# Snoworday/instance-segmentation-attention

Measured on AMD Instinct MI355X. Metric: images/sec @256x256 bs=16 per GPU, higher is better.
Workload: dtype bf16; 1 GPU; train.py step fwd+bwd+update 256x256 bs=16/GPU (bf16); global_batch=16, parallelism=dp1, launch=hipGraph replay

## Files before the change

### instance-segmentation-attention_amd/csrc/conv_fused_bwd.hip

```cpp
#include "common.hpp"
#include "tr_lds.hpp"

int wgrad_slab_reduce_launch(float* ws, float* dw, float* dbias, int gx, int tn, int tk, int N, int cin, int taps,
                             isa_slab_arena* sa, hipStream_t s);

namespace {

struct PwParams {
    const bf16_t *g, *y, *x; bf16_t* dx; const float* w; float* dw;
    int N, K, ldg, ldy, ldx, lddx; long M;
    const float *ysc, *ysh, *ymu, *yis, *yred; float ycnt_inv; int yact; float *ydgamma, *ydbeta;
    const float *xsc, *xsh, *xmu, *xis; int xact; float* xred;
    int accumulate; float* ws;
    const bf16_t* addend; int lda;
    int G;
};

#ifdef ISA_PHASE_TRACE
__device__ unsigned long long phase_buf[10];
#endif

template <int TN, int TK, int YACT, int XMODE, bool EPI>
__global__ __launch_bounds__(256) __attribute__((amdgpu_waves_per_eu(2, 2))) void pw_bn_bwd_kernel(PwParams p) {
    extern __shared__ __attribute__((aligned(16))) char ldsb[];
    PHASE_DECL(); PHASE(0);
    constexpr int PMB = 32;
    constexpr int SN = TrStride<TN * 32>::bytes, SK = TrStride<TK * 32>::bytes;
    constexpr int SLAB = PMB * (SN + SK);
    constexpr int VN = TN * 4, VK = TK * 4;
    constexpr int LOADS_N = PMB * VN / 64, LOADS_K = PMB * VK / 64;
    constexpr int RPN = 64 / VN, RPK = 64 / VK;
    constexpr int XACT = XMODE == 1 ? ISA_ACT_RELU6 : (XMODE == 0 ? ISA_ACT_NONE : ACT_RT);
    constexpr int NS = TN * 2;
    const int tid = threadIdx.x, wave = tid >> 6, lane = tid & 63;
    const int r = lane & 31, hh = lane >> 5;
    char* sD = ldsb + wave * SLAB;
    char* sX = sD + PMB * SN;
    const GroupSel gs = group_sel(p.G);
    if (gs.g) {
        const long gm = (long)gs.g * p.M;
        p.g += gm * p.ldg; p.y += gm * p.ldy; p.x += gm * p.ldx; p.dx += gm * p.lddx;
        if (p.addend) p.addend += gm * p.lda;
        p.ysc += gs.g * p.N; p.ysh += gs.g * p.N; p.ymu += gs.g * p.N; p.yis += gs.g * p.N; p.yred += gs.g * ISA_STAT_R * 2 * p.N;
        p.xsc = goff(p.xsc, (long)gs.g * p.K); p.xsh = goff(p.xsh, (long)gs.g * p.K); p.xmu = goff(p.xmu, (long)gs.g * p.K);
        p.xis = goff(p.xis, (long)gs.g * p.K); p.xred = goff(p.xred, (long)gs.g * ISA_STAT_R * 2 * p.K);
    }
    const bool want_xred = XMODE == 1 || (XMODE == 2 && p.xred != nullptr);

    const int cgn = lane % VN, rown = lane / VN, cgk = lane % VK, rowk = lane / VK;
    const int cn0 = cgn * 8, ck0 = cgk * 8;
    const bool nok = cn0 < p.N, kok = ck0 < p.K;
    const int cnl = nok ? cn0 : 0, ckl = kok ? ck0 : 0;

    bf16x8 rg[LOADS_N], ry[LOADS_N], rx[LOADS_K], rxc[LOADS_K];
    const long nchunks = (p.M + PMB - 1) / PMB;
    auto fetch = [&](long chunk) {
        const long mbase = chunk * PMB;
#pragma unroll
        for (int v = 0; v < LOADS_N; ++v) {
            const long m = min(mbase + v * RPN + rown, p.M - 1);
            rg[v] = *reinterpret_cast<const bf16x8*>(p.g + m * p.ldg + cnl);
            ry[v] = *reinterpret_cast<const bf16x8*>(p.y + m * p.ldy + cnl);
        }
#pragma unroll
        for (int v = 0; v < LOADS_K; ++v) {
            const long m = min(mbase + v * RPK + rowk, p.M - 1);
            rx[v] = *reinterpret_cast<const bf16x8*>(p.x + m * p.ldx + ckl);
        }
    };
    const long stride = (long)gs.nbx * 4;
    long chunk = (long)gs.bx * 4 + wave;
    if (chunk < nchunks) fetch(chunk);

    float* cst = reinterpret_cast<float*>(ldsb + 4 * SLAB);
    constexpr int WP = TN * 32 + 8;
    bf16_t* wl = reinterpret_cast<bf16_t*>(ldsb);
    float wv[TN * TK * 4];
#pragma unroll
    for (int it = 0; it < TN * TK * 4; ++it) {
        const int i = it * 256 + tid, n = i / (TK * 32), k = i % (TK * 32);
        wv[it] = p.w[min(n, p.N - 1) * p.K + min(k, p.K - 1)];
    }
    if (tid < 64) {
        const int cn = min(tid, p.N - 1), ck = min(tid, p.K - 1);
        cst[0 * 64 + tid] = p.ysc[cn]; cst[1 * 64 + tid] = p.ysh[cn]; cst[2 * 64 + tid] = p.ymu[cn];
        float r0 = 0.f, r1 = 0.f;
#pragma unroll
        for (int r = 0; r < ISA_STAT_R; ++r) { r0 += p.yred[r * 2 * p.N + cn]; r1 += p.yred[r * 2 * p.N + p.N + cn]; }
        cst[3 * 64 + tid] = p.yis[cn] * (r1 * p.ycnt_inv);
        cst[4 * 64 + tid] = r0 * p.ycnt_inv;
        if (gs.bx == 0 && tid < p.N) {
            if (p.ydgamma) atomicAdd(p.ydgamma + tid, r1);
            if (p.ydbeta) atomicAdd(p.ydbeta + tid, r0);
        }
        cst[5 * 64 + tid] = (XMODE && p.xsc) ? p.xsc[ck] : 1.f; cst[6 * 64 + tid] = (XMODE && p.xsh) ? p.xsh[ck] : 0.f;
        cst[7 * 64 + tid] = (XMODE && p.xmu) ? p.xmu[ck] : 0.f; cst[8 * 64 + tid] = (XMODE && p.xis) ? p.xis[ck] : 1.f;
    }
#pragma unroll
    for (int it = 0; it < TN * TK * 4; ++it) {
        const int i = it * 256 + tid, n = i / (TK * 32), k = i % (TK * 32);
        wl[k * WP + n] = (bf16_t)((n < p.N && k < p.K) ? wv[it] : 0.f);
    }
    __syncthreads();
    PHASE(1);
    auto ldc = [&](int which, int c0, float (&v)[8]) {
        const f32x4 a = *reinterpret_cast<const f32x4*>(cst + which * 64 + c0), b = *reinterpret_cast<const f32x4*>(cst + which * 64 + c0 + 4);
#pragma unroll
        for (int j = 0; j < 4; ++j) { v[j] = a[j]; v[4 + j] = b[j]; }
    };
    bf16x8 wb[NS][TK];
#pragma unroll
    for (int s = 0; s < NS; ++s)
#pragma unroll
        for (int j = 0; j < TK; ++j)
            wb[s][j] = *reinterpret_cast<const bf16x8*>(wl + (32 * j + r) * WP + 16 * s + 8 * hh);
    __syncthreads();
    PHASE(2);

    f32x16 acc[TN][TK];
#pragma unroll
    for (int i = 0; i < TN; ++i)
#pragma unroll
        for (int j = 0; j < TK; ++j) acc[i][j] = f32x16{0};
    float s0[8], s1[8];
#pragma unroll
    for (int j = 0; j < 8; ++j) { s0[j] = 0.f; s1[j] = 0.f; }

    auto stash = [&](long chunk) {
        const long mbase = chunk * PMB;
        {
        float ysc[8], ysh[8], ymu[8], yq[8], yk0[8];
        ldc(0, cn0, ysc); ldc(1, cn0, ysh); ldc(2, cn0, ymu); ldc(3, cn0, yq); ldc(4, cn0, yk0);
#pragma unroll
        for (int v = 0; v < LOADS_N; ++v) {
            const bool ok = (mbase + v * RPN + rown) < p.M && nok;
            bf16x8 o;
#pragma unroll
            for (int j = 0; j < 8; ++j) {
                const float yy = (float)ry[v][j];
                const float dz = (float)rg[v][j] * act_grad_t<YACT>(fmaf(yy, ysc[j], ysh[j]), p.yact);
                const float val = ysc[j] * (dz - yk0[j] - (yy - ymu[j]) * yq[j]);
                o[j] = (bf16_t)((ok && cn0 + j < p.N) ? val : 0.f);
            }
            *reinterpret_cast<bf16x8*>(sD + (v * RPN + rown) * SN + cgn * 16) = o;
        }
        }
        float xsc[8], xsh[8];
        ldc(5, ck0, xsc); ldc(6, ck0, xsh);
#pragma unroll
        for (int v = 0; v < LOADS_K; ++v) {
            const bool ok = (mbase + v * RPK + rowk) < p.M && kok;
            bf16x8 o;
#pragma unroll
            for (int j = 0; j < 8; ++j) {
                const float xr = (float)rx[v][j];
                const float z = XMODE ? act_t<XACT>(fmaf(xr, xsc[j], xsh[j]), p.xact) : xr;
                o[j] = (bf16_t)((ok && ck0 + j < p.K) ? z : 0.f);
            }
            *reinterpret_cast<bf16x8*>(sX + (v * RPK + rowk) * SK + cgk * 16) = o;
            rxc[v] = rx[v];
        }
    };

    for (; chunk < nchunks; chunk += stride) {
        stash(chunk);
        __builtin_amdgcn_fence(__ATOMIC_RELEASE, "wavefront");
        __builtin_amdgcn_wave_barrier();
        PHASE_ONCE(3);
        constexpr bool EPI_PREFETCH = EPI && TK == 1;
        bf16x8 repi_old[EPI_PREFETCH ? LOADS_K : 1], repi_add[EPI_PREFETCH ? LOADS_K : 1];
        if constexpr (EPI_PREFETCH) {
            const long mb = chunk * PMB;
#pragma unroll
            for (int v = 0; v < LOADS_K; ++v) {
                const long m = min(mb + v * RPK + rowk, p.M - 1);
                repi_old[v] = bf16x8{0}; repi_add[v] = bf16x8{0};
                if (p.accumulate) repi_old[v] = *reinterpret_cast<const bf16x8*>(p.dx + m * p.lddx + ckl);
                if (p.addend) repi_add[v] = *reinterpret_cast<const bf16x8*>(p.addend + m * p.lda + ckl);
            }
        }
        if (chunk + stride < nchunks) fetch(chunk + stride);
#pragma unroll
        for (int s = 0; s < PMB / 16; ++s) {
            bf16x8 a[TN], b[TK];
#pragma unroll
            for (int i = 0; i < TN; ++i) a[i] = tr_frag(sD, SN, 16 * s, i * 32, lane);
#pragma unroll
            for (int j = 0; j < TK; ++j) b[j] = tr_frag(sX, SK, 16 * s, j * 32, lane);
#pragma unroll
            for (int i = 0; i < TN; ++i)
#pragma unroll
                for (int j = 0; j < TK; ++j)
                    acc[i][j] = __builtin_amdgcn_mfma_f32_32x32x16_bf16(a[i], b[j], acc[i][j], 0, 0, 0);
        }
        f32x16 dxa[TK];
#pragma unroll
        for (int j = 0; j < TK; ++j) dxa[j] = f32x16{0};
#pragma unroll
        for (int s = 0; s < NS; ++s) {
            const bf16x8 a = *reinterpret_cast<const bf16x8*>(sD + r * SN + (16 * s + 8 * hh) * 2);
#pragma unroll
            for (int j = 0; j < TK; ++j)
                dxa[j] = __builtin_amdgcn_mfma_f32_32x32x16_bf16(a, wb[s][j], dxa[j], 0, 0, 0);
        }
        __builtin_amdgcn_fence(__ATOMIC_RELEASE, "wavefront");
        __builtin_amdgcn_wave_barrier();
#pragma unroll
        for (int j = 0; j < TK; ++j)
#pragma unroll
            for (int e = 0; e < 16; ++e) {
                const int row = (e & 3) + 8 * (e >> 2) + 4 * hh;
                *reinterpret_cast<bf16_t*>(sX + row * SK + (32 * j + r) * 2) = (bf16_t)dxa[j][e];
            }
        __builtin_amdgcn_fence(__ATOMIC_RELEASE, "wavefront");
        __builtin_amdgcn_wave_barrier();
        const long mbase = chunk * PMB;
        float xsc[8], xsh[8], xmu[8], xis[8];
        if (want_xred) { ldc(5, ck0, xsc); ldc(6, ck0, xsh); ldc(7, ck0, xmu); ldc(8, ck0, xis); }
#pragma unroll
        for (int v = 0; v < LOADS_K; ++v) {
            const long m = mbase + v * RPK + rowk;
            if (m < p.M && kok) {
                bf16x8 o = *reinterpret_cast<const bf16x8*>(sX + (v * RPK + rowk) * SK + cgk * 16);
                bf16_t* dst = p.dx + m * p.lddx + ck0;
                if constexpr (EPI) {
                    if (p.accumulate) {
                        bf16x8 old;
                        if constexpr (EPI_PREFETCH) old = repi_old[v]; else old = *reinterpret_cast<const bf16x8*>(dst);
#pragma unroll
                        for (int j = 0; j < 8; ++j) o[j] = (bf16_t)((float)o[j] + (float)old[j]);
                    }
                    if (p.addend) {
                        bf16x8 ad;
                        if constexpr (EPI_PREFETCH) ad = repi_add[v]; else ad = *reinterpret_cast<const bf16x8*>(p.addend + m * p.lda + ck0);
#pragma unroll
                        for (int j = 0; j < 8; ++j) o[j] = (bf16_t)((float)o[j] + (float)ad[j]);
                    }
                }
                *reinterpret_cast<bf16x8*>(dst) = o;
                if (want_xred) {
#pragma unroll
                    for (int j = 0; j < 8; ++j) {
                        const float xr = (float)rxc[v][j];
                        const float dz = (float)o[j] * act_grad_t<XACT>(fmaf(xr, xsc[j], xsh[j]), p.xact);
                        s0[j] += dz; s1[j] += dz * ((xr - xmu[j]) * xis[j]);
                    }
                }
            }
        }
        __builtin_amdgcn_fence(__ATOMIC_RELEASE, "wavefront");
        __builtin_amdgcn_wave_barrier();
    }

    PHASE(4);
    __syncthreads();
    PHASE(5);
    float* part = reinterpret_cast<float*>(ldsb);
    float* xs = part + fold_part_floats<TN, TK>();
    fold_park<TN, TK>(part, acc, wave, lane);
    if (want_xred) {
        float* slot = xs + (wave * 4 + (lane >> 4)) * (2 * TK * 32);
#pragma unroll
        for (int j = 0; j < 8; ++j) {
            const float v0 = row_fold<VK>(s0[j]), v1 = row_fold<VK>(s1[j]);
            if ((lane & 15) < VK) { slot[ck0 + j] = v0; slot[TK * 32 + ck0 + j] = v1; }
        }
    }
    __syncthreads();
    PHASE(6);
    constexpr int SLABF = TN * TK * 1024 + TN * 32;
    float* slab = p.ws + (long)blockIdx.x * SLABF;
    fold_store<TN, TK>(part, slab, tid);
    PHASE(7);
    if (tid < TN * 32) slab[TN * TK * 1024 + tid] = 0.f;
    if (want_xred && tid < 2 * TK * 32) {
        float v = 0.f;
#pragma unroll
        for (int sl = 0; sl < 16; ++sl) v += xs[sl * (2 * TK * 32) + tid];
        const int which = tid / (TK * 32), c = tid - which * TK * 32;
        if (c < p.K && v != 0.f)
            atomicAdd(p.xred + (blockIdx.x & (ISA_STAT_R - 1)) * 2 * p.K + which * p.K + c, v);
    }
    PHASE(8);
    PHASE_FLUSH(phase_buf);
}

template <int TN, int TK, int YACT, int XMODE>
int launch_inst(PwParams& p, long ws_floats, isa_slab_arena* sa, const isa_pro* xfin, int xfin_groups, hipStream_t s) {
    constexpr int SN = TrStride<TN * 32>::bytes, SK = TrStride<TK * 32>::bytes;
    constexpr size_t slab = (size_t)32 * (SN + SK) * 4 + 9 * 64 * 4;
    constexpr size_t redb = ((size_t)fold_part_floats<TN, TK>() + 16 * 2 * TK * 32) * 4;
    constexpr size_t lds = slab > redb ? slab : redb;
    const long nchunks = (p.M + 31) / 32;
    const long slabf = (long)TN * TK * 1024 + TN * 32;
    long gx = (nchunks + 3) / 4 * p.G;
    if (gx > 256 * 2) gx = 256 * 2;
    if (int rc = defer_ws(sa, &p.ws, &ws_floats)) return rc;
    const long ws_cap = ws_floats / slabf;
    if (ws_cap < p.G) return sa ? ISA_ENOMEM : ISA_EINVAL;
    if (gx > ws_cap) gx = ws_cap;
    gx = group_grid(gx, p.G);
    if (int rc = fin_standalone(xfin, p.K, xfin_groups, s)) return rc;
    if (p.accumulate || p.addend) hipLaunchKernelGGL((pw_bn_bwd_kernel<TN, TK, YACT, XMODE, true>), dim3((unsigned)gx), dim3(256), lds, s, p);
    else hipLaunchKernelGGL((pw_bn_bwd_kernel<TN, TK, YACT, XMODE, false>), dim3((unsigned)gx), dim3(256), lds, s, p);
    if (launch_status() != ISA_OK) return ISA_ELAUNCH;
    return wgrad_slab_reduce_launch(p.ws, p.dw, nullptr, (int)gx, TN, TK, p.N, p.K, 1, sa, s);
}

template <int TN, int TK>
int launch_tile(PwParams& p, int xmode, long ws_floats, isa_slab_arena* sa, const isa_pro* xfin, int xfin_groups, hipStream_t s) {
    const bool y6 = p.yact == ISA_ACT_RELU6, y0 = p.yact == ISA_ACT_NONE;
#define PW_X(YA) (xmode == 0 ? launch_inst<TN, TK, YA, 0>(p, ws_floats, sa, xfin, xfin_groups, s) \
                : xmode == 1 ? launch_inst<TN, TK, YA, 1>(p, ws_floats, sa, xfin, xfin_groups, s) \
                             : launch_inst<TN, TK, YA, 2>(p, ws_floats, sa, xfin, xfin_groups, s))
    if (y6) return PW_X(ISA_ACT_RELU6);
    if (y0) return PW_X(ISA_ACT_NONE);
    return PW_X(ACT_RT);
#undef PW_X
}

}

#ifdef ISA_PHASE_TRACE
extern "C" int isa_phase_trace_pw(unsigned long long* out) { return hipMemcpyFromSymbol(out, HIP_SYMBOL(phase_buf), sizeof(phase_buf)) == hipSuccess ? ISA_OK : ISA_ELAUNCH; }
#endif

extern "C" int isa_conv1x1_bn_backward(const isa_tensor* g, const isa_tensor* y, const isa_bn_bwd* ybn,
                                       const isa_tensor* x, const isa_pro* xpro, const isa_bn_bwd* xbn,
                                       const float* w, float* dw, const isa_tensor* dx, int32_t accumulate,
                                       const isa_tensor* addend, float* ws, int64_t ws_floats, isa_slab_arena* defer,
                                       void* stream) {
    if (!tensor_ok(g, 8) || !tensor_ok(y, 8) || !tensor_ok(x, 8) || !tensor_ok(dx, 8)) return ISA_EINVAL;
    if (!fin_valid(xpro)) return ISA_EINVAL;
    if (g->dtype != ISA_BF16 || y->dtype != ISA_BF16 || x->dtype != ISA_BF16 || dx->dtype != ISA_BF16) return ISA_EINVAL;
    if (!ybn || !ybn->scale || !ybn->shift || !ybn->mean || !ybn->invstd || !ybn->red || !(ybn->count > 0)) return ISA_EINVAL;
    if (!w || !dw || (!ws && !defer)) return ISA_EINVAL;
    const int N = g->c, K = x->c;
    if (N > 64 || K > 64 || N % 8 || K % 8) return ISA_EINVAL;
    if (y->c != N || dx->c != K) return ISA_EINVAL;
    const isa_tensor* ts[3] = {y, x, dx};
    for (const isa_tensor* t : ts)
        if (t->n != g->n || t->h != g->h || t->w != g->w) return ISA_EINVAL;
    const ProDev xp = make_pro(xpro);
    if (xp.bscale) return ISA_EINVAL;
    if (xbn && (!xbn->mean || !xbn->invstd || !xbn->out_red)) return ISA_EINVAL;
    PwParams p{};
    p.g = (const bf16_t*)g->data; p.y = (const bf16_t*)y->data; p.x = (const bf16_t*)x->data; p.dx = (bf16_t*)dx->data;
    p.w = w; p.dw = dw; p.N = N; p.K = K; p.ldg = g->ld; p.ldy = y->ld; p.ldx = x->ld; p.lddx = dx->ld;
    p.G = tensor_groups(g);
    if (g->n % p.G) return ISA_EINVAL;
    p.M = (long)(g->n / p.G) * g->h * g->w;
    p.ysc = ybn->scale; p.ysh = ybn->shift; p.ymu = ybn->mean; p.yis = ybn->invstd; p.yred = ybn->red;
    p.ycnt_inv = 1.f / ybn->count; p.yact = ybn->act; p.ydgamma = ybn->dgamma; p.ydbeta = ybn->dbeta;
    p.xsc = xp.scale; p.xsh = xp.shift; p.xact = xp.act;
    p.xmu = xbn ? xbn->mean : nullptr; p.xis = xbn ? xbn->invstd : nullptr; p.xred = xbn ? xbn->out_red : nullptr;
    p.accumulate = accumulate; p.ws = ws;
    if (addend) {
        if (!tensor_ok(addend, 8) || addend->dtype != ISA_BF16 || addend->c != K || addend->n != g->n || addend->h != g->h ||
            addend->w != g->w) return ISA_EINVAL;
        p.addend = (const bf16_t*)addend->data; p.lda = addend->ld;
    }
    int xmode = 0;
    if (!pro_trivial(xp) || xbn) xmode = (xbn && xp.act == ISA_ACT_RELU6) ? 1 : 2;
    hipStream_t s = as_stream(stream);
    const int tn = (N + 31) / 32, tk = (K + 31) / 32;
    if (tn == 1 && tk == 1) return launch_tile<1, 1>(p, xmode, ws_floats, defer, xpro, tensor_groups(x), s);
    if (tn == 1 && tk == 2) return launch_tile<1, 2>(p, xmode, ws_floats, defer, xpro, tensor_groups(x), s);
    if (tn == 2 && tk == 1) return launch_tile<2, 1>(p, xmode, ws_floats, defer, xpro, tensor_groups(x), s);
    return launch_tile<2, 2>(p, xmode, ws_floats, defer, xpro, tensor_groups(x), s);
}
```

### instance-segmentation-attention_amd/engine.py

```python
import contextlib
import ctypes as C
import os
from typing import Dict, List, Optional, Tuple

import torch

from . import lib as L


STAT_R = 8


def rup(x, m):
    return (x + m - 1) // m * m


class PendingFin:
    __slots__ = ("eng", "stats", "count", "pre", "c", "scale", "shift", "mean", "invstd", "groups", "rep", "running_taken",
                 "done", "keep")

    def __init__(self, eng, stats, count, pre, c, scale, shift, mean, invstd, groups, rep, running_taken):
        self.eng, self.stats, self.count, self.pre, self.c = eng, stats, count, pre, c
        self.scale, self.shift, self.mean, self.invstd, self.groups, self.rep = scale, shift, mean, invstd, groups, rep
        self.running_taken = running_taken
# ... 338 lines not shown

    def mark_sync(self, src, dst):
        list.append(self, (None, (src, dst)))

    def last_fn(self):
        return self[-1][0] if (self and self[-1][0] is not None) else Tape


class GradBook:

    def __init__(self, eng):
        self.eng = eng
        self.bufs: Dict[int, torch.Tensor] = {}
        self.written: Dict[int, List[Tuple[int, int]]] = {}

    def reset(self):
        self.bufs.clear()
        self.written.clear()
        self.shared: Dict[int, torch.Tensor] = {}

    def share(self, a: Act):
        self.shared[a.buf.data_ptr()] = a.buf

    def _key(self, a: Act):
        p = a.buf.data_ptr()
        cur = self.eng.cur
        return (p, cur) if (cur != 0 and p in self.shared) else p

    def grad_of(self, a: Act) -> Act:
        key = self._key(a)
        g = self.bufs.get(key)
        if g is None:
            g = self.eng.arena.alloc(a.buf.shape, a.buf.dtype)
            self.bufs[key] = g
            self.written[key] = []
        return Act(g, a.c0, a.c, groups=a.groups)

    def _covered(self, key, lo, hi):
        segs = sorted(self.written[key])
        missing, cur = [], lo
        for s, e in segs:
            if e <= cur:
                continue
            if s >= hi:
                break
            if s > cur:
                missing.append((cur, min(s, hi)))
            cur = max(cur, e)
            if cur >= hi:
                break
        if cur < hi:
            missing.append((cur, hi))
        full = not missing
        none = len(missing) == 1 and missing[0] == (lo, hi)
        return full, none, missing

    def claim(self, a: Act, eng) -> int:
        key = self._key(a)
        if key not in self.bufs:
            self.grad_of(a)
        lo, hi = a.c0, a.c0 + a.c
        full, none, missing = self._covered(key, lo, hi)
        if not full:
            self.written[key].append((lo, hi))
        if full:
            return 1
        if none:
            return 0
        g = self.bufs[key]
        for s, e in missing:
            eng.fill_zero(Act(g, s, e - s))
        return 1

    def has(self, a: Act) -> bool:
        key = self._key(a)
        if key not in self.bufs:
            return False
        full, _, _ = self._covered(key, a.c0, a.c0 + a.c)
        return full

    def merge_shared(self, eng):
        assert eng.cur == 0
        for key in [k for k in self.bufs if isinstance(k, tuple)]:
            p, _ = key
            side = self.bufs[key]
            segs, merged = sorted(self.written[key]), []
            for lo, hi in segs:
                if merged and lo <= merged[-1][1]:
                    merged[-1][1] = max(merged[-1][1], hi)
                else:
                    merged.append([lo, hi])
            for lo, hi in merged:
                a = Act(self.shared[p], lo, hi - lo)
                acc = self.claim(a, eng)
                eng.lib.isa_axpy(Act(side, lo, hi - lo).d(), self.grad_of(a).d(), 1.0, acc, eng.st())
            self.written[key] = []


class _ProfiledLib:

    def __init__(self, lib, eng):
        self._lib, self._eng = lib, eng
        self._cache = {}

    def __getattr__(self, name):
        fn = getattr(self._lib, name)
        eng = self._eng

        def call(*args):
            if not eng.profile:
                return fn(*args)
            s = torch.cuda.Event(enable_timing=True)
            e = torch.cuda.Event(enable_timing=True)
            s.record()
            rc = fn(*args)
            e.record()
            eng.prof_events.append((name, s, e, eng.next_bytes))
            eng.next_bytes = 0
            return rc

        self._cache[name] = call
        setattr(self, name, call)
        return call


class Engine:
    BN_EPS = 1e-5
    BN_MOMENTUM = 0.1

    def __init__(self, params: ParamStore, dtype=torch.float32, device="cuda"):
        self.params = params
        self.dtype = dtype
        self.device = device
        self.packer = Packer(params, dtype)
        self.arenas: Dict[object, Arena] = {}
        self.arena = self.arenas.setdefault(None, Arena(device))
        self.grads = GradBook(self)
        self.tape = Tape(self)
        self.cur = 0
        self.side_streams: Dict[int, torch.cuda.Stream] = {}
        self.main_stream = None
        self.defer_bn_running = False
        self.bn_running_queue: List[tuple] = []
        self.bn_train = False
        self.record = False
        self.lib = _ProfiledLib(L.checked(), self)
        self.ws = torch.empty(16 << 20, dtype=torch.float32, device=device)
        self.profile = False
        self.prof_events = []
        self.next_bytes = 0
        self.fuse_dw_bn = os.environ.get("ISA_FUSE_DW_BN", "1") != "0"
        self._dw_out: Dict[tuple, ConvFusion] = {}
        self.fuse_pw_bn = os.environ.get("ISA_FUSE_PW_BN", "1") != "0"
        self.fuse_eval = os.environ.get("ISA_FUSE_EVAL", "1") != "0"
        self.fuse_block = os.environ.get("ISA_FUSE_BLOCK", "1") != "0"
        self.inline_fin = os.environ.get("ISA_INLINE_FIN", "1") != "0"
        self._pw_out: Dict[tuple, ConvFusion] = {}
        self._pw_in: Dict[tuple, ConvFusion] = {}
        self.eval_bn_cache: Dict[str, tuple] = {}
        self.eval_bn_stale = False
        self.fold_arena = None
        self.slab = None
        self.fold_stats = (0, 0)
        self._deferring = False
        self.defer_fold = os.environ.get("ISA_DEFER_FOLD", "1") != "0"
        self.bn_repeat = 1
        self.arena_cache = int(os.environ.get("ISA_ARENA_CACHE", "4"))
        self._eval_bn_ready: Dict[str, tuple] = {}

    def begin(self, bn_train: bool, record: bool, key=None):
        akey = (bool(bn_train), bool(record), key)
        arena = self.arenas.pop(akey, None)
        if arena is None:
            arena = Arena(self.device)
        self.arenas[akey] = arena
        loose = [k for k, a in self.arenas.items() if not a.frozen and k != akey and k is not None]
        for k in loose[:max(0, len(loose) - self.arena_cache)]:
            del self.arenas[k]
        self.arena = arena
        arena.reset()
        if POISON:
            self.ws.view(torch.uint8).fill_(0xFF)
        self.grads.reset()
        self.tape = Tape(self)
        self.cur = 0
        self.main_stream = torch.cuda.current_stream()
        self.defer_bn_running = False
        self.bn_running_queue = []
        self._dw_out = {}
        self._pw_out = {}
        self._pw_in = {}
        self.bn_train, self.record = bn_train, record
        if not bn_train and self.eval_bn_stale:
            self.refresh_eval_bn()

    def freeze_arena(self):
        self.arena.frozen = True

    def _stream(self, sid):
        if sid == 0:
            return self.main_stream
        st = self.side_streams.get(sid)
        if st is None:
            st = self.side_streams[sid] = torch.cuda.Stream(device=self.device)
        return st

    @contextlib.contextmanager
    def on(self, sid):
        prev = self.cur
        self.cur = sid
        try:
            if sid == 0:
                with torch.cuda.stream(self.main_stream):
                    yield
            else:
                assert self.defer_fold or not self.record, "concurrent branches need the slab arena (ISA_DEFER_FOLD=1)"
                with torch.cuda.stream(self._stream(sid)):
                    yield
        finally:
            self.cur = prev

    def _wait(self, src, dst):
        if src == dst:
            return
        ev = torch.cuda.Event()
        ev.record(self._stream(src))
        self._stream(dst).wait_event(ev)

    def sync(self, src, dst):
        if src != 0 and dst != 0 and src != dst:
            raise RuntimeError("Engine.sync(%d, %d): stream edges must have the step's own stream (0) at one end - "
                               "side-to-side edges crash hipGraph capture on ROCm 7.2" % (src, dst))
        self._wait(src, dst)
        if self.record:
            self.tape.mark_sync(src, dst)

    def flush_bn_running(self):
        q = self.bn_running_queue
        if not q:
            return
        P = self.params
        runs, seen = [[]], set()
        for ent in q:
            if ent[2] in seen:
                runs.append([]); seen = set()
            seen.add(ent[2]); runs[-1].append(ent)
        for run in runs:
            arr = (L.IsaBnUpd * len(run))()
            for i, (stats, count, pre, c) in enumerate(run):
                arr[i] = L.IsaBnUpd(stats.data_ptr(), P.ptr(pre + ".running_mean").value, P.ptr(pre + ".running_var").value,
                                    count, c)
            self.lib.isa_bn_running_update(arr, len(run), self.BN_MOMENTUM, self.st())
        self.bn_running_queue = []

    def running_ptrs(self, pre):
        P = self.params
        return P.ptr(pre + ".running_mean"), P.ptr(pre + ".running_var")

    def bn_finalize(self, stats, count, pre, running, scale, shift, mean, invstd, c, groups, rep):
        P = self.params
        rm, rv = running or (None, None)
        self.lib.isa_bn_finalize(stats, count, P.ptr(pre + ".weight"), P.ptr(pre + ".bias"), rm, rv, self.BN_MOMENTUM,
                                 self.BN_EPS, scale, shift, mean, invstd, c, groups, rep, self.st())

    def _finalize_train(self, stats, count, pre, c, scale, shift, mean, invstd, groups=1):
        defer = self.defer_bn_running
        rep = self.bn_repeat
        assert not (defer and (groups > 1 or rep > 1)), "deferred running statistics are a single-group mechanism"
        fin = None
        if self.inline_fin:
            fin = PendingFin(self, stats, count, pre, c, scale, shift, mean, invstd, groups, rep, running_taken=defer)
        else:
            self.bn_finalize(stats, count, pre, None if defer else self.running_ptrs(pre), scale, shift, mean, invstd,
                             c, groups, rep)
        if defer:
            self.bn_running_queue.append((stats, count, pre, c))
        self.params.int_buffers[pre + ".num_batches_tracked"] += groups * rep
        return fin

    def defer_handle(self):
        return self.slab if (self._deferring and self.defer_fold) else None

    def _eval_bn_filled(self, pre):
        ev = torch.cuda.Event()
        ev.record(torch.cuda.current_stream())
        self._eval_bn_ready[pre] = (ev, self.cur)

    def _eval_bn_wait(self, pre):
        ent = self._eval_bn_ready.get(pre)
        if ent is not None and ent[1] != self.cur and not torch.cuda.is_current_stream_capturing():
            torch.cuda.current_stream().wait_event(ent[0])

    def refresh_eval_bn(self):
        for pre, consts in self.eval_bn_cache.items():
            self.bn_finalize(None, 1.0, pre, self.running_ptrs(pre), *consts, consts[0].numel(), 1, 1)
        self.eval_bn_stale = False

    def scratch(self, numel) -> torch.Tensor:
        return self.arena.scratch(numel)

    def f32(self, *shape):
        return self.arena.alloc(shape, torch.float32)

    def new_act(self, n, h, w, c, ld=None, dtype=None, groups=1):
        ld = rup(c, 8) if ld is None else ld
        return Act(self.arena.alloc((n, h, w, ld), dtype or self.dtype), 0, c, groups=groups)
# ... 14 lines not shown
        return L.stream_ptr()

    def fill_zero(self, a: Act):
        self.lib.isa_axpy(a.d(), a.d(), 0.0, 0, self.st())

    def copy(self, src: Act, dst: Act):
        self.lib.isa_axpy(src.d(), dst.d(), 1.0, 0, self.st())
        if self.record and src.needs_grad:
            def bwd():
                acc = self.grads.claim(src, self)
                self.lib.isa_axpy(self.grads.grad_of(dst).d(), self.grads.grad_of(src).d(), 1.0, acc, self.st())
            self.tape.append(bwd)

    def reg_conv(self, wname, taps=1, kmap=None, transposed=False):
        shape = self.params.shapes[wname]
        if transposed:
            k, co = shape[0], shape[1]
            kphys = len(kmap) if kmap is not None else k
            kp = rup(kphys, 32)
            f = self.packer.add(wname, "fwd", 2, co, k, 4, kp, 4 * co, kmap)
            b = self.packer.add(wname, "dgrad", 3, co, k, 4, rup(co, 32), kphys, kmap)
            return dict(fwd=f, dgrad=b, kp=kp, kp_d=rup(co, 32), n=4 * co, kphys=kphys)
        n, k = shape[0], shape[1]
        kphys = len(kmap) if kmap is not None else k
        kp = rup(kphys, 32)
        f = self.packer.add(wname, "fwd", 0, n, k, taps, kp, n, kmap)
        b = self.packer.add(wname, "dgrad", 1, n, k, taps, rup(n, 32), kphys, kmap)
        return dict(fwd=f, dgrad=b, kp=kp, kp_d=rup(n, 32), n=n, kphys=kphys)

    def eval_fusable(self):
        return self.fuse_eval and not self.bn_train and not self.record

    def eval_bn(self, pre, c):
        cached = self.eval_bn_cache.get(pre)
        if cached is None:
            cached = tuple(torch.empty(c, dtype=torch.float32, device=self.device) for _ in range(4))
            self.eval_bn_cache[pre] = cached
            self.bn_finalize(None, 1.0, pre, self.running_ptrs(pre), *cached, c, 1, 1)
            self._eval_bn_filled(pre)
        else:
            self._eval_bn_wait(pre)
        return cached

    def conv_bn_eval(self, x: Act, wname, out: Act, bn_pre, act, res: Optional[Act] = None, taps=1):
        assert self.eval_fusable()
        reg = self.reg_conv(wname, taps, None, False)
        if self.packer.table is None:
            self.packer.pack()
        scale, shift, _, _ = self.eval_bn(bn_pre, out.c)
        if self.profile:
            esz = x.buf.element_size()
            self.next_bytes = (x.n * x.h * x.w * x.c + (1 + (res is not None)) * out.n * out.h * out.w * out.c) * esz
        ep = L.IsaConvEp(L.addr(scale), L.addr(shift), act, C.addressof(res._c) if res is not None else None)
        self._keep_ep = (ep, res)
        self.lib.isa_conv_gemm_ep(x.d(), x.p(), self.packer.ptr(reg["fwd"]), reg["kp"], None, out.d(),
                                  L.IN_3X3 if taps == 9 else L.IN_1X1, C.byref(ep), self.st())
        return out

    def block_v1_eval_fusable(self, x: Act, cout):
        return (self.fuse_block and self.eval_fusable() and self.dtype == torch.bfloat16 and x.pro is None and x.c % 32 == 0
                and x.c <= 128 and cout % 16 == 0 and cout <= 64 and x.h % 8 == 0 and x.w % 32 == 0 and x.ld % 8 == 0)

    def block_v1_eval(self, x: Act, pre, out: Act, res: Optional[Act] = None):
        rd = self.reg_dw(pre + ".conv.0.weight")
        rc = self.reg_conv(pre + ".conv.3.weight")
        if self.packer.table is None:
            self.packer.pack()
        s1, h1, _, _ = self.eval_bn(pre + ".conv.1", x.c)
        s2, h2, _, _ = self.eval_bn(pre + ".conv.4", out.c)
        if self.profile:
            esz = x.buf.element_size()
            self.next_bytes = (x.n * x.h * x.w * x.c + (1 + (res is not None)) * out.n * out.h * out.w * out.c) * esz
        ep = L.IsaConvEp(L.addr(s2), L.addr(h2), L.ACT_NONE, C.addressof(res._c) if res is not None else None)
        self._keep_ep = (ep, res)
        self.lib.isa_dwpw_eval(x.d(), self.packer.ptr(rd["fwd"]), s1, h1, self.packer.ptr(rc["fwd"]), rc["kp"], C.byref(ep),
                               out.d(), self.st())
        return out

    def conv(self, x: Act, wname, out: Act, *, taps=1, bias=None, stats=False, kmap=None,
             transposed=False, record_bwd=True):
        reg = self.reg_conv(wname, taps, kmap, transposed)
        in_mode = L.IN_3X3 if taps == 9 else L.IN_1X1
        out_mode = L.OUT_SHUFFLE2 if transposed else L.OUT_PLAIN
        st = self.scratch(2 * out.c * STAT_R * out.groups) if stats else None
        job = (x, reg, bias, out, in_mode, out_mode, st)
        self._launch_conv(*job)
        if self.record and record_bwd:
            rec = None
            if self.fuse_pw_bn and self.bn_train and self.dtype == torch.bfloat16 and taps == 1 and not transposed \
                    and kmap is None and bias is None and x.needs_grad and out.c <= 64 and x.c <= 64 \
                    and out.c % 8 == 0 and x.c % 8 == 0 and (x.pro is None or x.pro.bscale is None):
                rec = self._pw_out[self._key(out)] = self._pw_in[self._key(x)] = ConvFusion(self._bn_just_recorded(x))
            wshape = self.params.shapes[wname]
            wg_in, ksrc = (L.IN_1X1, wshape[0]) if transposed else (in_mode, wshape[1])

            def bwd():
                if rec is not None:
                    rec.done = True
                    if rec.ybn is not None:
                        self._fused_pw_backward(x, wname, rec)
                        return
                    self._flush_addend(x, rec)
                dy = self.grads.grad_of(out)
                pk = self.packer
                if self.profile and not transposed:
                    self.next_bytes = (x.n * x.h * x.w * x.c + dy.n * dy.h * dy.w * dy.c) * x.buf.element_size()
                self.lib.isa_conv_wgrad(x.d(), x.p(), dy.d(), self.params.gptr(wname),
                                        self.params.gptr(bias) if bias else None, wg_in, out_mode, pk.kmap_ptr(reg["fwd"]),
                                        ksrc, self.ws, self.ws.numel(), self.defer_handle(), self.st())
                if x.needs_grad:
                    acc = self.grads.claim(x, self)
                    dx = self.grads.grad_of(x)
                    if transposed:
                        self.lib.isa_conv_gemm(dy.d(), None, pk.ptr(reg["dgrad"]), reg["kp_d"], None, dx.d(), L.IN_GATHER2,
                                               L.OUT_PLAIN, None, acc, self.st())
                    else:
                        if self.profile:
                            self.next_bytes = (dy.n * dy.h * dy.w * dy.c + dx.n * dx.h * dx.w * dx.c) * dy.buf.element_size()
                        self.lib.isa_conv_gemm(dy.d(), None, pk.ptr(reg["dgrad"]), reg["kp_d"], None, dx.d(), in_mode,
                                               L.OUT_PLAIN, None, acc, self.st())
            self.tape.append(bwd)
        return out, st

    def _bn_desc(self, b, red=None, out_red=None, with_params=True):
        P = self.params
        return L.IsaBnBwd(L.addr(b.scale), L.addr(b.shift), L.addr(b.mean), L.addr(b.invstd), L.addr(red), L.addr(out_red),
                          P.gptr(b.pre + ".weight").value if with_params else None,
                          P.gptr(b.pre + ".bias").value if with_params else None, b.count, b.act)

    @staticmethod
    def _key(a: Act):
        return (a.buf.data_ptr(), a.c0, a.c)

    def _bn_just_recorded(self, x: Act):
        xb = x.bn
        return xb if (xb is not None and xb.train and self.tape.last_fn() is xb.bwd_fn) else None

    def _fused_descs(self, x: Act, rec):
        ydesc, xdesc = self._bn_desc(rec.ybn, red=rec.yred), None
        if rec.xbn is not None:
            rec.xbn.red_done = self.scratch(2 * x.c * STAT_R * x.groups)
            xdesc = self._bn_desc(rec.xbn, out_red=rec.xbn.red_done, with_params=False)
        return ydesc, xdesc

    def _flush_addend(self, x: Act, rec):
        if rec.addend is not None:
            acc = self.grads.claim(x, self)
            self.lib.isa_axpy(rec.addend.d(), self.grads.grad_of(x).d(), 1.0, acc, self.st())

    def _fused_pw_backward(self, x: Act, wname, rec):
        ydesc, xdesc = self._fused_descs(x, rec)
        acc = self.grads.claim(x, self)
        g = rec.g
        if self.profile:
            self.next_bytes = x.n * x.h * x.w * (2 * g.c + 2 * x.c) * x.buf.element_size()
        self.lib.isa_conv1x1_bn_backward(g.d(), rec.ybn.raw.d(), C.byref(ydesc), x.d(), x.p(),
                                         C.byref(xdesc) if xdesc is not None else None, self.params.ptr(wname),
                                         self.params.gptr(wname), self.grads.grad_of(x).d(), acc,
                                         rec.addend.d() if rec.addend is not None else None, self.ws, self.ws.numel(),
                                         self.defer_handle(), self.st())

    def _launch_conv(self, x, reg, bias, out, in_mode, out_mode, st):
        if self.packer.table is None:
            self.packer.pack()
        if self.profile:
            esz = x.buf.element_size()
            self.next_bytes = (x.n * x.h * x.w * x.c + out.n * out.h * out.w * out.c) * esz
        self.lib.isa_conv_gemm(x.d(), x.p_fin(), self.packer.ptr(reg["fwd"]), reg["kp"],
                               self.params.ptr(bias) if bias else None, out.d(), in_mode, out_mode, st, 0, self.st())

    def reg_dw(self, wname, kmap=None):
        c = self.params.shapes[wname][0]
        rows = rup(len(kmap) if kmap is not None else c, 8)
        f = self.packer.add(wname, "fwd", 4, c, 1, 9, 0, rows, kmap)
        b = self.packer.add(wname, "dgrad", 5, c, 1, 9, 0, rows, kmap)
        return dict(fwd=f, dgrad=b)

    def dwconv(self, x: Act, wname, out: Act, *, bias=None, stats=False, kmap=None):
        reg = self.reg_dw(wname, kmap)
        if self.packer.table is None:
            self.packer.pack()
        st = self.scratch(2 * out.c * STAT_R * out.groups) if stats else None
        if self.profile:
            self.next_bytes = 2 * x.n * x.h * x.w * x.c * x.buf.element_size()
        self.lib.isa_dwconv3x3(x.d(), x.p_fin(), self.packer.ptr(reg["fwd"]), self.params.ptr(bias) if bias else None,
                               out.d(), st, self.st())
        if self.record:
            rec = None
            if self.fuse_dw_bn and self.bn_train and x.c % 8 == 0 and bias is None and x.needs_grad \
                    and (x.pro is None or x.pro.bscale is None):
                rec = self._dw_out[self._key(out)] = ConvFusion(self._bn_just_recorded(x))
                if x.pro is None and x.bn is None:
                    self._pw_in.setdefault(self._key(x), rec)

            def bwd():
                dy = self.grads.grad_of(out)
                nb = x.n * x.h * x.w * x.c * x.buf.element_size()
                if rec is not None:
                    rec.done = True
                    if rec.ybn is not None:
                        ydesc, xdesc = self._fused_descs(x, rec)
                        acc = self.grads.claim(x, self)
                        if self.profile:
                            self.next_bytes = 4 * nb
                        self.lib.isa_dwconv3x3_bn_backward(dy.d(), rec.ybn.raw.d(), C.byref(ydesc), x.d(), x.p(),
                                                           C.byref(xdesc) if xdesc is not None else None,
                                                           self.packer.ptr(reg["dgrad"]), self.params.gptr(wname),
                                                           self.params.shapes[wname][0], self.grads.grad_of(x).d(), acc,
                                                           rec.addend.d() if rec.addend is not None else None, self.ws,
                                                           self.ws.numel(), self.defer_handle(), self.st())
                        return
                    self._flush_addend(x, rec)
                if self.profile:
                    self.next_bytes = 2 * nb
                self.lib.isa_dwconv3x3_wgrad(x.d(), x.p(), dy.d(), self.params.gptr(wname),
                                             self.params.gptr(bias) if bias else None, self.params.shapes[wname][0],
                                             self.ws, self.ws.numel(), self.defer_handle(), self.st())
                if x.needs_grad:
                    acc = self.grads.claim(x, self)
                    if self.profile:
                        self.next_bytes = 2 * nb
                    self.lib.isa_dwconv3x3_dgrad(dy.d(), self.packer.ptr(reg["dgrad"]), self.grads.grad_of(x).d(), acc,
                                                 self.st())
            self.tape.append(bwd)
        return out, st

    def _bn_layer(self, raw: Act, stats, pre, act, count):
        c, G = raw.c, raw.groups
        count = float(raw.n // G * raw.h * raw.w) if count is None else float(count)
        train = self.bn_train
        assert train or G == 1, "statistic groups exist in train mode only (eval statistics are shared)"
        fin = None
        if train:
            scale, shift, mean, invstd = (self.f32(G * c) for _ in range(4))
            fin = self._finalize_train(stats, count, pre, c, scale, shift, mean, invstd, G)
        else:
            scale, shift, mean, invstd = self.eval_bn(pre, c)
        return BnLayer(pre, scale, shift, mean, invstd, act, count, train, raw), fin

    def bn(self, raw: Act, stats, pre, act, count=None) -> Act:
        b, fin = self._bn_layer(raw, stats, pre, act, count)
        lazy = raw.with_pro(Pro(b.scale, b.shift, act, fin=fin))
        lazy.bn = b
        if self.record:
            rec = None
            if b.train:
                key = self._key(raw)
                rec = self._dw_out.get(key)
                if rec is None:
                    rec = self._pw_out.get(key)

            def bwd():
                g = self.grads.grad_of(raw)
                if rec is not None:
                    rec.ybn, rec.yred, rec.g = b, self._bn_backward(lazy, g, g, None, do_apply=False), g
                    return
                self._bn_backward(lazy, g, g, None)
            b.bwd_fn = bwd
            self.tape.append(bwd)
        return lazy

    def _bn_backward(self, lazy: Act, dt: Act, dy: Act, bscale, do_apply=True):
        b = lazy.bn
        P = self.params
        red, b.red_done = b.red_done, None
        nb = lazy.n * lazy.h * lazy.w * lazy.c * lazy.buf.element_size()
        if red is None:
            red = self.scratch(2 * lazy.c * STAT_R * lazy.groups)
            if self.profile:
                self.next_bytes = 2 * nb
            self.lib.isa_bn_bwd_reduce(dt.d(), b.raw.d(), b.scale, b.shift, b.mean, b.invstd, b.act, bscale, red, self.st())
        if not do_apply:
            return red
        if self.profile:
            self.next_bytes = 3 * nb
        self.lib.isa_bn_bwd_apply(dt.d(), b.raw.d(), b.scale, b.shift, b.mean, b.invstd, b.act, bscale,
                                  P.ptr(b.pre + ".weight"), red, b.count, 1 if b.train else 0, dy.d(),
                                  P.gptr(b.pre + ".weight"), P.gptr(b.pre + ".bias"), self.st())
        return red

    def bn_out(self, raw: Act, stats, pre, act, out: Act, res: Optional[Act] = None, bscale=None,
               count=None, res2: Optional[Act] = None, oscale=None) -> Act:
        b, fin = self._bn_layer(raw, stats, pre, act, count)
        lazy = raw.with_pro(Pro(b.scale, b.shift, act, bscale, fin=fin))
        lazy.bn = b
        if self.profile:
            self.next_bytes = (2 + (res is not None) + (res2 is not None)) * raw.n * raw.h * raw.w * raw.c * raw.buf.element_size()
        self.lib.isa_affine_act_res(lazy.d(), lazy.p_fin(), res.d() if res is not None else None,
                                    res2.d() if res2 is not None else None, oscale, out.d(), self.st())
        if self.record:
            pw = self._pw_out.get(self._key(raw)) if (b.train and bscale is None) else None

            bcast = out.n != raw.n
            assert not bcast or (oscale is not None and res2 is None and out.n == out.groups * raw.n and raw.groups == 1)

            def bwd():
                dout = self.grads.grad_of(out)
                dsum = dout
                if oscale is not None:
                    dsum = self.like(raw, out.c)
                    self.lib.isa_scale_bc(dout.d(), oscale, dsum.d(), 0, self.st())
                for r in (res, res2):
                    if r is not None and r.needs_grad:
                        pin = self._pw_in.get(self._key(r))
                        if pin is not None and not pin.done and pin.addend is None:
                            pin.addend = dsum
                            continue
                        acc = self.grads.claim(r, self)
                        self.lib.isa_axpy(dsum.d(), self.grads.grad_of(r).d(), 1.0, acc, self.st())
# ... 80 lines not shown
```

Measured before the change: 726.4 images/s.

## Recompute pointwise conv output in fused BN backward instead of reading it

For 1x1 conv + BN backward with ReLU6 or no activation and small channel counts, the kernel no longer loads the pre-BN conv output y from global memory. It recomputes y per chunk with an extra MFMA of x against the weights held in registers or LDS, then applies the BN/activation gradient in LDS. This trades one activation read stream for extra matrix math, LDS traffic and register pressure. The recomputed y is rounded to bf16 to match the stored value.

New measurement: 737.1 images/s, median of 6. 1.01x the previous value.

```diff
diff --git a/instance-segmentation-attention_amd/csrc/conv_fused_bwd.hip b/instance-segmentation-attention_amd/csrc/conv_fused_bwd.hip
--- a/instance-segmentation-attention_amd/csrc/conv_fused_bwd.hip
+++ b/instance-segmentation-attention_amd/csrc/conv_fused_bwd.hip
@@ -20,7 +20,28 @@
 __device__ unsigned long long phase_buf[10];
 #endif
 
-template <int TN, int TK, int YACT, int XMODE, bool EPI>
+template <int YACT>
+__device__ __forceinline__ float bn_bwd_dy(float g, float yy, float sc, float sh, float mu, float q, float k0, int rt) {
+    const float dz = g * act_grad_t<YACT>(fmaf(yy, sc, sh), rt);
+    return sc * (dz - k0 - (yy - mu) * q);
+}
+
+template <int HS>
+__device__ __forceinline__ bf16x8 tr_frag_h(const char* tile, int stride_bytes, int row0, int col0, int lane) {
+    const int g = lane >> 4, i = lane & 15, q = i >> 2, pp = i & 3;
+    const char* a = tile + (row0 + HS * (g >> 1) + q) * stride_bytes + (col0 + 16 * (g & 1) + 4 * pp) * 2;
+    const s16x4 lo = __builtin_amdgcn_ds_read_tr16_b64_v4i16(LDS_S16X4(a));
+    const s16x4 hi = __builtin_amdgcn_ds_read_tr16_b64_v4i16(LDS_S16X4(a + 4 * stride_bytes));
+    const s16x8 v = __builtin_shufflevector(lo, hi, 0, 1, 2, 3, 4, 5, 6, 7);
+    return __builtin_bit_cast(bf16x8, v);
+}
+
+template <int WP>
+__device__ __forceinline__ bf16x8 rec_wfrag(const bf16_t* wl, int s, int i, int lane) {
+    return tr_frag_h<16>(reinterpret_cast<const char*>(wl), WP * 2, 32 * (s >> 1) + 8 * (s & 1), i * 32, lane);
+}
+
+template <int TN, int TK, int YACT, int XMODE, bool EPI, bool REC>
 __global__ __launch_bounds__(256) __attribute__((amdgpu_waves_per_eu(2, 2))) void pw_bn_bwd_kernel(PwParams p) {
     extern __shared__ __attribute__((aligned(16))) char ldsb[];
     PHASE_DECL(); PHASE(0);
@@ -39,7 +60,9 @@
     const GroupSel gs = group_sel(p.G);
     if (gs.g) {
         const long gm = (long)gs.g * p.M;
-        p.g += gm * p.ldg; p.y += gm * p.ldy; p.x += gm * p.ldx; p.dx += gm * p.lddx;
+        p.g += gm * p.ldg;
+        if constexpr (!REC) p.y += gm * p.ldy;
+        p.x += gm * p.ldx; p.dx += gm * p.lddx;
         if (p.addend) p.addend += gm * p.lda;
         p.ysc += gs.g * p.N; p.ysh += gs.g * p.N; p.ymu += gs.g * p.N; p.yis += gs.g * p.N; p.yred += gs.g * ISA_STAT_R * 2 * p.N;
         p.xsc = goff(p.xsc, (long)gs.g * p.K); p.xsh = goff(p.xsh, (long)gs.g * p.K); p.xmu = goff(p.xmu, (long)gs.g * p.K);
@@ -52,7 +75,7 @@
     const bool nok = cn0 < p.N, kok = ck0 < p.K;
     const int cnl = nok ? cn0 : 0, ckl = kok ? ck0 : 0;
 
-    bf16x8 rg[LOADS_N], ry[LOADS_N], rx[LOADS_K], rxc[LOADS_K];
+    bf16x8 rg[LOADS_N], ry[REC ? 1 : LOADS_N], rx[LOADS_K], rxc[LOADS_K];
     const long nchunks = (p.M + PMB - 1) / PMB;
     auto fetch = [&](long chunk) {
         const long mbase = chunk * PMB;
@@ -60,7 +83,7 @@
         for (int v = 0; v < LOADS_N; ++v) {
             const long m = min(mbase + v * RPN + rown, p.M - 1);
             rg[v] = *reinterpret_cast<const bf16x8*>(p.g + m * p.ldg + cnl);
-            ry[v] = *reinterpret_cast<const bf16x8*>(p.y + m * p.ldy + cnl);
+            if constexpr (!REC) ry[v] = *reinterpret_cast<const bf16x8*>(p.y + m * p.ldy + cnl);
         }
 #pragma unroll
         for (int v = 0; v < LOADS_K; ++v) {
@@ -74,7 +97,8 @@
 
     float* cst = reinterpret_cast<float*>(ldsb + 4 * SLAB);
     constexpr int WP = TN * 32 + 8;
-    bf16_t* wl = reinterpret_cast<bf16_t*>(ldsb);
+    constexpr bool WLDS = REC && TN * TK == 4;
+    bf16_t* wl = reinterpret_cast<bf16_t*>(WLDS ? ldsb + 4 * SLAB + 9 * 64 * 4 : ldsb);
     float wv[TN * TK * 4];
 #pragma unroll
     for (int it = 0; it < TN * TK * 4; ++it) {
@@ -114,6 +138,14 @@
 #pragma unroll
         for (int j = 0; j < TK; ++j)
             wb[s][j] = *reinterpret_cast<const bf16x8*>(wl + (32 * j + r) * WP + 16 * s + 8 * hh);
+    constexpr bool WREG = REC && !WLDS;
+    bf16x8 wf[WREG ? 2 * TK : 1][WREG ? TN : 1];
+    if constexpr (WREG) {
+#pragma unroll
+        for (int s = 0; s < 2 * TK; ++s)
+#pragma unroll
+            for (int i = 0; i < TN; ++i) wf[s][i] = rec_wfrag<WP>(wl, s, i, lane);
+    }
     __syncthreads();
     PHASE(2);
 
@@ -128,7 +160,10 @@
 
     auto stash = [&](long chunk) {
         const long mbase = chunk * PMB;
-        {
+        if constexpr (REC) {
+#pragma unroll
+            for (int v = 0; v < LOADS_N; ++v) *reinterpret_cast<bf16x8*>(sD + (v * RPN + rown) * SN + cgn * 16) = rg[v];
+        } else {
         float ysc[8], ysh[8], ymu[8], yq[8], yk0[8];
         ldc(0, cn0, ysc); ldc(1, cn0, ysh); ldc(2, cn0, ymu); ldc(3, cn0, yq); ldc(4, cn0, yk0);
 #pragma unroll
@@ -180,6 +215,35 @@
             }
         }
         if (chunk + stride < nchunks) fetch(chunk + stride);
+        if constexpr (REC) {
+            const int rows = (int)min((long)PMB, p.M - chunk * PMB) - 4 * hh;
+#pragma unroll
+            for (int i = 0; i < TN; ++i) {
+                f32x16 ya = f32x16{0};
+#pragma unroll
+                for (int s = 0; s < 2 * TK; ++s) {
+                    const bf16x8 a = *reinterpret_cast<const bf16x8*>(sX + r * SK + (32 * (s >> 1) + 16 * hh + 8 * (s & 1)) * 2);
+                    bf16x8 b;
+                    if constexpr (WLDS) b = rec_wfrag<WP>(wl, s, i, lane); else b = wf[s][i];
+                    ya = __builtin_amdgcn_mfma_f32_32x32x16_bf16(a, b, ya, 0, 0, 0);
+                }
+                const int n = 32 * i + r;
+                const float ysc = cst[0 * 64 + n], ysh = cst[1 * 64 + n], ymu = cst[2 * 64 + n], yq = cst[3 * 64 + n], yk0 = cst[4 * 64 + n];
+                const unsigned colm = n < p.N ? 0xffffu : 0u;
+                unsigned short* d = reinterpret_cast<unsigned short*>(sD + 4 * hh * SN + n * 2);
+                unsigned short gr[16];
+#pragma unroll
+                for (int e = 0; e < 16; ++e) gr[e] = d[((e & 3) + 8 * (e >> 2)) * (SN / 2)];
+#pragma unroll
+                for (int e = 0; e < 16; ++e) {
+                    const float val = bn_bwd_dy<YACT>(__uint_as_float((unsigned)gr[e] << 16), (float)(bf16_t)ya[e], ysc, ysh, ymu, yq, yk0, p.yact);
+                    const unsigned o = __builtin_bit_cast(unsigned short, (bf16_t)val);
+                    d[((e & 3) + 8 * (e >> 2)) * (SN / 2)] = (unsigned short)(o & ((e & 3) + 8 * (e >> 2) < rows ? colm : 0u));
+                }
+            }
+            __builtin_amdgcn_fence(__ATOMIC_RELEASE, "wavefront");
+            __builtin_amdgcn_wave_barrier();
+        }
 #pragma unroll
         for (int s = 0; s < PMB / 16; ++s) {
             bf16x8 a[TN], b[TK];
@@ -285,12 +349,13 @@
     PHASE_FLUSH(phase_buf);
 }
 
-template <int TN, int TK, int YACT, int XMODE>
+template <int TN, int TK, int YACT, int XMODE, bool REC>
 int launch_inst(PwParams& p, long ws_floats, isa_slab_arena* sa, const isa_pro* xfin, int xfin_groups, hipStream_t s) {
     constexpr int SN = TrStride<TN * 32>::bytes, SK = TrStride<TK * 32>::bytes;
     constexpr size_t slab = (size_t)32 * (SN + SK) * 4 + 9 * 64 * 4;
     constexpr size_t redb = ((size_t)fold_part_floats<TN, TK>() + 16 * 2 * TK * 32) * 4;
-    constexpr size_t lds = slab > redb ? slab : redb;
+    constexpr size_t wkeep = (REC && TN * TK == 4) ? (size_t)TK * 32 * (TN * 32 + 8) * 2 : 0;
+    constexpr size_t lds = slab + wkeep > redb ? slab + wkeep : redb;
     const long nchunks = (p.M + 31) / 32;
     const long slabf = (long)TN * TK * 1024 + TN * 32;
     long gx = (nchunks + 3) / 4 * p.G;
@@ -301,8 +366,8 @@
     if (gx > ws_cap) gx = ws_cap;
     gx = group_grid(gx, p.G);
     if (int rc = fin_standalone(xfin, p.K, xfin_groups, s)) return rc;
-    if (p.accumulate || p.addend) hipLaunchKernelGGL((pw_bn_bwd_kernel<TN, TK, YACT, XMODE, true>), dim3((unsigned)gx), dim3(256), lds, s, p);
-    else hipLaunchKernelGGL((pw_bn_bwd_kernel<TN, TK, YACT, XMODE, false>), dim3((unsigned)gx), dim3(256), lds, s, p);
+    if (p.accumulate || p.addend) hipLaunchKernelGGL((pw_bn_bwd_kernel<TN, TK, YACT, XMODE, true, REC>), dim3((unsigned)gx), dim3(256), lds, s, p);
+    else hipLaunchKernelGGL((pw_bn_bwd_kernel<TN, TK, YACT, XMODE, false, REC>), dim3((unsigned)gx), dim3(256), lds, s, p);
     if (launch_status() != ISA_OK) return ISA_ELAUNCH;
     return wgrad_slab_reduce_launch(p.ws, p.dw, nullptr, (int)gx, TN, TK, p.N, p.K, 1, sa, s);
 }
@@ -310,12 +375,12 @@
 template <int TN, int TK>
 int launch_tile(PwParams& p, int xmode, long ws_floats, isa_slab_arena* sa, const isa_pro* xfin, int xfin_groups, hipStream_t s) {
     const bool y6 = p.yact == ISA_ACT_RELU6, y0 = p.yact == ISA_ACT_NONE;
-#define PW_X(YA) (xmode == 0 ? launch_inst<TN, TK, YA, 0>(p, ws_floats, sa, xfin, xfin_groups, s) \
-                : xmode == 1 ? launch_inst<TN, TK, YA, 1>(p, ws_floats, sa, xfin, xfin_groups, s) \
-                             : launch_inst<TN, TK, YA, 2>(p, ws_floats, sa, xfin, xfin_groups, s))
-    if (y6) return PW_X(ISA_ACT_RELU6);
-    if (y0) return PW_X(ISA_ACT_NONE);
-    return PW_X(ACT_RT);
+#define PW_X(YA, RC) (xmode == 0 ? launch_inst<TN, TK, YA, 0, RC>(p, ws_floats, sa, xfin, xfin_groups, s) \
+                    : xmode == 1 ? launch_inst<TN, TK, YA, 1, RC>(p, ws_floats, sa, xfin, xfin_groups, s) \
+                                 : launch_inst<TN, TK, YA, 2, RC>(p, ws_floats, sa, xfin, xfin_groups, s))
+    if (y6) return p.y ? PW_X(ISA_ACT_RELU6, false) : PW_X(ISA_ACT_RELU6, true);
+    if (y0) return p.y ? PW_X(ISA_ACT_NONE, false) : PW_X(ISA_ACT_NONE, true);
+    return PW_X(ACT_RT, false);
 #undef PW_X
 }
 
@@ -330,23 +395,24 @@
                                        const float* w, float* dw, const isa_tensor* dx, int32_t accumulate,
                                        const isa_tensor* addend, float* ws, int64_t ws_floats, isa_slab_arena* defer,
                                        void* stream) {
-    if (!tensor_ok(g, 8) || !tensor_ok(y, 8) || !tensor_ok(x, 8) || !tensor_ok(dx, 8)) return ISA_EINVAL;
+    if (!tensor_ok(g, 8) || (y && !tensor_ok(y, 8)) || !tensor_ok(x, 8) || !tensor_ok(dx, 8)) return ISA_EINVAL;
     if (!fin_valid(xpro)) return ISA_EINVAL;
-    if (g->dtype != ISA_BF16 || y->dtype != ISA_BF16 || x->dtype != ISA_BF16 || dx->dtype != ISA_BF16) return ISA_EINVAL;
+    if (g->dtype != ISA_BF16 || (y && y->dtype != ISA_BF16) || x->dtype != ISA_BF16 || dx->dtype != ISA_BF16) return ISA_EINVAL;
     if (!ybn || !ybn->scale || !ybn->shift || !ybn->mean || !ybn->invstd || !ybn->red || !(ybn->count > 0)) return ISA_EINVAL;
     if (!w || !dw || (!ws && !defer)) return ISA_EINVAL;
+    if (!y && ybn->act != ISA_ACT_RELU6 && ybn->act != ISA_ACT_NONE) return ISA_EINVAL;
     const int N = g->c, K = x->c;
     if (N > 64 || K > 64 || N % 8 || K % 8) return ISA_EINVAL;
-    if (y->c != N || dx->c != K) return ISA_EINVAL;
+    if ((y && y->c != N) || dx->c != K) return ISA_EINVAL;
     const isa_tensor* ts[3] = {y, x, dx};
     for (const isa_tensor* t : ts)
-        if (t->n != g->n || t->h != g->h || t->w != g->w) return ISA_EINVAL;
+        if (t && (t->n != g->n || t->h != g->h || t->w != g->w)) return ISA_EINVAL;
     const ProDev xp = make_pro(xpro);
     if (xp.bscale) return ISA_EINVAL;
     if (xbn && (!xbn->mean || !xbn->invstd || !xbn->out_red)) return ISA_EINVAL;
     PwParams p{};
-    p.g = (const bf16_t*)g->data; p.y = (const bf16_t*)y->data; p.x = (const bf16_t*)x->data; p.dx = (bf16_t*)dx->data;
-    p.w = w; p.dw = dw; p.N = N; p.K = K; p.ldg = g->ld; p.ldy = y->ld; p.ldx = x->ld; p.lddx = dx->ld;
+    p.g = (const bf16_t*)g->data; p.y = y ? (const bf16_t*)y->data : nullptr; p.x = (const bf16_t*)x->data; p.dx = (bf16_t*)dx->data;
+    p.w = w; p.dw = dw; p.N = N; p.K = K; p.ldg = g->ld; p.ldy = y ? y->ld : 0; p.ldx = x->ld; p.lddx = dx->ld;
     p.G = tensor_groups(g);
     if (g->n % p.G) return ISA_EINVAL;
     p.M = (long)(g->n / p.G) * g->h * g->w;
diff --git a/instance-segmentation-attention_amd/engine.py b/instance-segmentation-attention_amd/engine.py
--- a/instance-segmentation-attention_amd/engine.py
+++ b/instance-segmentation-attention_amd/engine.py
@@ -514,6 +514,7 @@
         self.fuse_dw_bn = os.environ.get("ISA_FUSE_DW_BN", "1") != "0"
         self._dw_out: Dict[tuple, ConvFusion] = {}
         self.fuse_pw_bn = os.environ.get("ISA_FUSE_PW_BN", "1") != "0"
+        self.pw_recompute = os.environ.get("ISA_PW_RECOMPUTE", "1") != "0"
         self.fuse_eval = os.environ.get("ISA_FUSE_EVAL", "1") != "0"
         self.fuse_block = os.environ.get("ISA_FUSE_BLOCK", "1") != "0"
         self.inline_fin = os.environ.get("ISA_INLINE_FIN", "1") != "0"
@@ -834,9 +835,10 @@
         ydesc, xdesc = self._fused_descs(x, rec)
         acc = self.grads.claim(x, self)
         g = rec.g
+        y = None if (self.pw_recompute and rec.ybn.act in (L.ACT_RELU6, L.ACT_NONE) and min(g.c, x.c) <= 32) else rec.ybn.raw.d()
         if self.profile:
-            self.next_bytes = x.n * x.h * x.w * (2 * g.c + 2 * x.c) * x.buf.element_size()
-        self.lib.isa_conv1x1_bn_backward(g.d(), rec.ybn.raw.d(), C.byref(ydesc), x.d(), x.p(),
+            self.next_bytes = x.n * x.h * x.w * ((1 if y is None else 2) * g.c + 2 * x.c) * x.buf.element_size()
+        self.lib.isa_conv1x1_bn_backward(g.d(), y, C.byref(ydesc), x.d(), x.p(),
                                          C.byref(xdesc) if xdesc is not None else None, self.params.ptr(wname),
                                          self.params.gptr(wname), self.grads.grad_of(x).d(), acc,
                                          rec.addend.d() if rec.addend is not None else None, self.ws, self.ws.numel(),
```
